# meffmadd/intro-tc-vae

Hardware: AMD Instinct MI355X
Metric: images/sec (64x64x3, z=128, bs=64) intro-TC step (higher is better)
Workload: dtype f32 in/out/accumulate, conv products on split-fp16 MFMA (two scaled fp16 planes, 3 products, fp32-class); 1 GPU; c2: IntroTCSovler.train_step, conv arch, 64x64x3, z_dim=128, channels (64, 128, 256, 512), batch 64/GPU, Adam lr 2e-4, clip 100, N=10000; global_batch=64, parallelism=single, sync_bn=False

## Files before the change

### intro-tc-vae_amd/csrc/conv_igemm.hip

```cpp
#include <float.h>

#include "conv_shared.h"

namespace itcv {



constexpr uint32_t kOobBase = 0x80000000u;

__device__ __forceinline__ float buf_load_s(__amdgpu_buffer_rsrc_t r, uint32_t voff, uint32_t soff) {
  return __builtin_bit_cast(float, __builtin_amdgcn_raw_buffer_load_b32(r, voff, __builtin_amdgcn_readfirstlane(soff), 0));
}

__host__ __device__ inline int tile_rows_for(int M) { return M <= 32 ? 32 : (M <= 64 ? 64 : 128); }

struct ConvArgs {
  const float* x;
  const float* wp;
  const float* bias;
  float* y;
  int B, Ci, H, W, Co;
  int Cip, Mp, N;
  int mt, nt;
  int ktiles, ktiles_per_split, cpt;
// ... 205 lines not shown
    for (int i = 0; i < 8; ++i) {
      const int k = B_KC ? (t & 31) : (t >> 6) + 4 * i, n = B_KC ? (t >> 5) + 8 * i : (t & 63);
      pb[i] = a.B + (long long)min(kb + k, a.K - 1) * a.sbk + (long long)min(n0 + n, a.N - 1) * a.sbn;
    }
#pragma unroll
    for (int i = 0; i < 8; ++i) areg[i] = *pa[i];
#pragma unroll
    for (int i = 0; i < 8; ++i) breg[i] = *pb[i];
    __builtin_amdgcn_sched_group_barrier(0x020, 16, 0);
  };
  auto store_tile = [&](int buf, int kt) {
    const int kb = kt * BK;
#pragma unroll
    for (int i = 0; i < 8; ++i) {
      const int k = A_KC ? (t & 31) : (t >> 6) + 4 * i, m = A_KC ? (t >> 5) + 8 * i : (t & 63);
      As[buf][k * PA + m] = (m0 + m < a.M && kb + k < a.K) ? areg[i] : 0.f;
    }
#pragma unroll
    for (int i = 0; i < 8; ++i) {
      const int k = B_KC ? (t & 31) : (t >> 6) + 4 * i, n = B_KC ? (t >> 5) + 8 * i : (t & 63);
      Bs[buf][k * PB + n] = (n0 + n < a.N && kb + k < a.K) ? breg[i] : 0.f;
    }
  };
  f32x16 acc[1][1];
#pragma unroll
  for (int r = 0; r < 16; ++r) acc[0][0][r] = 0.f;
  if (kt0 < kt1) {
    load_tile(kt0);
    store_tile(0, kt0);
    __syncthreads();
    int cur = 0;
    for (int kt = kt0; kt < kt1; ++kt) {
      const bool more = kt + 1 < kt1;
      if (more) load_tile(kt + 1);
      mfma_tile<BK, PA, PB, 1, 1>(&As[cur][half * PA + wm * 32 + l31], &Bs[cur][half * PB + wn * 32 + l31], acc);
      if (more) store_tile(cur ^ 1, kt + 1);
      __syncthreads();
      cur ^= 1;
    }
  }
  const int n = n0 + wn * 32 + l31;
  if (n >= a.N) return;
  float* out = a.C + (size_t)sk * a.slab_stride;
  const float bv = (a.bias && !a.slab_stride) ? a.bias[n] : 0.f;
#pragma unroll
  for (int r = 0; r < 16; ++r) {
    const int m = m0 + wm * 32 + (r & 3) + 8 * (r >> 2) + 4 * half;
    if (m < a.M) {
      float* q = out + (size_t)m * a.N + n;
      float v = acc[0][0][r] + bv;
      if constexpr (EPI == 1) v = v > 0.f ? v : v * a.slope;
      if constexpr (EPI == 2) v *= a.mask[(long long)m * a.ldm + n] > 0.f ? 1.f : a.slope;
      *q = a.accumulate ? *q + v : v;
    }
  }
}

__global__ void gemm64_reduce(const float* __restrict__ slab, const float* __restrict__ bias, float* __restrict__ C,
                              size_t total, int N, int splits, int accumulate) {
  for (size_t i = (size_t)blockIdx.x * blockDim.x + threadIdx.x; i < total; i += (size_t)gridDim.x * blockDim.x) {
    float s = fold_strided(0.f, slab + i, total, splits);
    if (bias) s += bias[i % N];
    C[i] = accumulate ? C[i] + s : s;
  }
}

template <int EPI>
__global__ void gemm64_reduce_epi(const float* __restrict__ slab, const float* __restrict__ bias, float* __restrict__ C,
                                  size_t total, int N, int splits, const float* __restrict__ mask, long long ldm,
                                  float slope) {
  for (size_t i = (size_t)blockIdx.x * blockDim.x + threadIdx.x; i < total; i += (size_t)gridDim.x * blockDim.x) {
    float s = fold_strided(0.f, slab + i, total, splits);
    if (bias) s += bias[i % N];
    if constexpr (EPI == 1) s = s > 0.f ? s : s * slope;
    if constexpr (EPI == 2) s *= mask[(long long)(i / N) * ldm + (long long)(i % N)] > 0.f ? 1.f : slope;
    C[i] = s;
  }
}

__global__ void pack_weight_kernel(const float* __restrict__ w, float* __restrict__ wp, int Co, int Ci, int KK,
                                   int for_dgrad, int C, int M, int Cip, int Mp) {
  const size_t total = (size_t)KK * Cip * Mp;
  for (size_t i = (size_t)blockIdx.x * blockDim.x + threadIdx.x; i < total; i += (size_t)gridDim.x * blockDim.x) {
    const int k = (int)(i / Mp), m = (int)(i - (size_t)k * Mp);
    const int kt = k >> 4, cib = kt / KK, tap = kt - cib * KK, c = cib * 16 + (k & 15);
    float v = 0.f;
    if (c < C && m < M)
      v = for_dgrad ? w[((size_t)c * Ci + m) * KK + (KK - 1 - tap)] : w[((size_t)m * Ci + c) * KK + tap];
    wp[i] = v;
  }
}


struct ConvArgsB {
  const float* x;
  const u32x4* wp;
  const float* bias;
  float* y;
  int B, Ci, H, W, Co;
  int Mp, N;
  int mt, nt;
  int ktiles, ktiles_per_split, cpt;
  uint32_t x_bytes;
  size_t slab_stride;
#ifdef ITCV_DIAG
  int ablate;
// ... 1376 lines not shown
  if (d.accumulate) {
    if (vec) {
#pragma unroll
      for (int q = 0; q < 9; ++q) {
        const float4 t = reinterpret_cast<const float4*>(dwp)[q];
        tot[4 * q] = t.x, tot[4 * q + 1] = t.y, tot[4 * q + 2] = t.z, tot[4 * q + 3] = t.w;
      }
    } else {
#pragma unroll
      for (int q = 0; q < 36; ++q) tot[q] = dwp[q];
    }
  } else {
#pragma unroll
    for (int q = 0; q < 36; ++q) tot[q] = 0.f;
  }
  for (int k = 0; k < d.nsrc; ++k) {
    const float* p = d.slab[k] + e;
    float acc[36];
#pragma unroll
    for (int q = 0; q < 36; ++q) acc[q] = 0.f;
    int sl = 0;
    for (; sl + 2 <= d.splits[k]; sl += 2) {
      float4 v[2][9];
#pragma unroll
      for (int u = 0; u < 2; ++u)
#pragma unroll
        for (int tp = 0; tp < 9; ++tp) v[u][tp] = *reinterpret_cast<const float4*>(p + (size_t)(sl + u) * stride + (size_t)tp * plane);
#pragma unroll
      for (int u = 0; u < 2; ++u)
#pragma unroll
        for (int tp = 0; tp < 9; ++tp)
          acc[tp] += v[u][tp].x, acc[9 + tp] += v[u][tp].y, acc[18 + tp] += v[u][tp].z, acc[27 + tp] += v[u][tp].w;
    }
    if (sl < d.splits[k]) {
      float4 v[9];
#pragma unroll
      for (int tp = 0; tp < 9; ++tp) v[tp] = *reinterpret_cast<const float4*>(p + (size_t)sl * stride + (size_t)tp * plane);
#pragma unroll
      for (int tp = 0; tp < 9; ++tp) acc[tp] += v[tp].x, acc[9 + tp] += v[tp].y, acc[18 + tp] += v[tp].z, acc[27 + tp] += v[tp].w;
    }
#pragma unroll
    for (int q = 0; q < 36; ++q) tot[q] += acc[q];
  }
  if (vec) {
#pragma unroll
    for (int q = 0; q < 9; ++q) reinterpret_cast<float4*>(dwp)[q] = make_float4(tot[4 * q], tot[4 * q + 1], tot[4 * q + 2], tot[4 * q + 3]);
  } else {
#pragma unroll
    for (int q = 0; q < 36; ++q) dwp[q] = tot[q];
  }
}

constexpr int kWgFineSplits = 64;
__device__ __forceinline__ void wgrad_reduce_tile_fine(const WgReduceDesc& d, int tile, float* part ) {
  const int lane = threadIdx.x & 63, wave = threadIdx.x >> 6, el = lane & 15, sg = wave * 4 + (lane >> 4);
  const int e0 = tile * 16, e = e0 + el;
  const bool live = e < d.coci;
  const size_t plane = (size_t)d.coci, stride = 9 * plane;
  const int o = threadIdx.x;
  const bool oo = o < 144 && e0 * 9 + o < d.coci * 9;
  float tot = (d.accumulate && oo) ? d.dw[(size_t)e0 * 9 + o] : 0.f;
  for (int k = 0; k < d.nsrc; ++k) {
    const int q = (d.splits[k] + 15) >> 4;
    const int s0 = sg * q, s1 = min(s0 + q, d.splits[k]);
    float acc[9];
#pragma unroll
    for (int tp = 0; tp < 9; ++tp) acc[tp] = 0.f;
    if (live) {
      const float* p = d.slab[k] + e;
      int sl = s0;
      for (; sl + 4 <= s1; sl += 4) {
        float v[4][9];
#pragma unroll
        for (int u = 0; u < 4; ++u)
#pragma unroll
          for (int tp = 0; tp < 9; ++tp) v[u][tp] = p[(size_t)(sl + u) * stride + (size_t)tp * plane];
#pragma unroll
        for (int u = 0; u < 4; ++u)
#pragma unroll
          for (int tp = 0; tp < 9; ++tp) acc[tp] += v[u][tp];
      }
      for (; sl < s1; ++sl) {
        float v[9];
#pragma unroll
        for (int tp = 0; tp < 9; ++tp) v[tp] = p[(size_t)sl * stride + (size_t)tp * plane];
#pragma unroll
        for (int tp = 0; tp < 9; ++tp) acc[tp] += v[tp];
      }
    }
    if (k) __syncthreads();
#pragma unroll
    for (int tp = 0; tp < 9; ++tp) part[(sg * 9 + tp) * 16 + el] = acc[tp];
    __syncthreads();
    if (o < 144) {
      const int el2 = o / 9, tp = o - el2 * 9;
      float sum = 0.f;
#pragma unroll
      for (int g = 0; g < 16; ++g) sum += part[(g * 9 + tp) * 16 + el2];
      tot += sum;
    }
  }
  if (oo) d.dw[(size_t)e0 * 9 + o] = tot;
}
static inline bool wgrad_reduce_fine(const int* splits, int nsrc) {
  for (int k = 0; k < nsrc; ++k)
    if (splits[k] >= kWgFineSplits) return true;
  return false;
}
static inline int wgrad_reduce_blocks(int coci, bool fine) { return fine ? cdiv(coci, 16) : cdiv(coci, 1024); }

__global__ __launch_bounds__(256) void wgrad_p_reduce(const float* __restrict__ slab, float* __restrict__ dw, int CoCi,
                                                     int splits, int accumulate, int fine) {
  __shared__ float part[4][9][64];
  WgReduceDesc d;
  d.slab[0] = slab, d.dw = dw, d.splits[0] = splits, d.nsrc = 1, d.coci = CoCi, d.accumulate = accumulate;
  if (fine) wgrad_reduce_tile_fine(d, blockIdx.x, &part[0][0][0]);
  else wgrad_reduce_tile(d, blockIdx.x);
}

constexpr int kWgMaxDesc = 96;
__global__ __launch_bounds__(256) void wgrad_p_reduce_many(const WgReduceDesc* __restrict__ tab, int n, int tile0, int tile1) {
  __shared__ float part[4][9][64];
  __shared__ WgReduceDesc s_desc[kWgMaxDesc];
  {
    const int* src = reinterpret_cast<const int*>(tab);
    int* dst = reinterpret_cast<int*>(s_desc);
    for (int i = threadIdx.x; i < n * (int)(sizeof(WgReduceDesc) / 4); i += blockDim.x) dst[i] = src[i];
  }
  __syncthreads();
  int di = 0;
  for (int t = tile0 + (int)blockIdx.x; t < tile1; t += (int)gridDim.x) {
    while (di + 1 < n && s_desc[di + 1].block0 <= t) ++di;
    const WgReduceDesc d = s_desc[di];
    if (d.fine) {
      wgrad_reduce_tile_fine(d, t - d.block0, &part[0][0][0]);
      __syncthreads();
    } else {
      wgrad_reduce_tile(d, t - d.block0);
    }
  }
}

__global__ __launch_bounds__(256) void splitk_reduce_wgrad_small(const float* __restrict__ slab, float* __restrict__ dw,
                                                                 int Co, int Ci, int KK, int Cip, int cb, int Np,
                                                                 size_t slab_stride, int splits, int accumulate,
                                                                 int swapped) {
  __shared__ float part[16][17];
  const int e = threadIdx.x & 15, g = threadIdx.x >> 4;
  const size_t total = (size_t)Co * Ci * KK, i = (size_t)blockIdx.x * 16 + e;
  float s = 0.f;
  if (i < total) {
    int tap = (int)(i % KK);
    const size_t r = i / KK;
    int ci = (int)(r % Ci), co = (int)(r / Ci);
    if (swapped) {
      const int tmp = ci;
      ci = co, co = tmp, tap = KK - 1 - tap;
    }
    int col;
    if (cb == 128) {
      const int per_tap = Cip / 128;
      col = (tap * per_tap + ci / 128) * 128 + (ci & 127);
    } else {
      const int tpb = 128 / cb;
      col = (tap / tpb) * 128 + (tap % tpb) * cb + ci;
    }
    const float* p = slab + (size_t)co * Np + col;
    for (int k = g; k < splits; k += 16) s += p[(size_t)k * slab_stride];
  }
  part[g][e] = s;
  __syncthreads();
  if (g == 0 && i < total) {
    float t = accumulate ? dw[i] : 0.f;
#pragma unroll
    for (int k = 0; k < 16; ++k) t += part[k][e];
    dw[i] = t;
  }
}

__global__ void splitk_reduce_wgrad(const float* __restrict__ slab, float* __restrict__ dw, int Co, int Ci, int KK,
                                    int Cip, int cb, int Np, size_t slab_stride, int splits, int accumulate,
                                    int swapped) {
  const size_t total = (size_t)Co * Ci * KK;
  for (size_t i = (size_t)blockIdx.x * blockDim.x + threadIdx.x; i < total; i += (size_t)gridDim.x * blockDim.x) {
    int tap = (int)(i % KK);
    const size_t r = i / KK;
    int ci = (int)(r % Ci), co = (int)(r / Ci);
    if (swapped) {
      const int tmp = ci;
      ci = co, co = tmp, tap = KK - 1 - tap;
    }
// ... 684 lines not shown
  ITCV_CHECK_LAUNCH("itcv_conv2d_wgrad_bf16s(reduce)");
  return 0;
}

int itcv_conv2d_wgrad_bf16p_supported(int B, int Ci, int H, int W, int Co, int KS) {
  if (KS != 3 || B <= 0 || Ci < 8 || Co < 8 || (Ci & 7) || (Co & 7)) return 0;
  if (log2_exact(W) < 2 || W > 256 || log2_exact(H) < 0) return 0;
  const long long px = (long long)B * H * W;
  if (px % 64) return 0;
  if (H * W < 64 && 64 % (H * W)) return 0;
  return 1;
}

size_t itcv_conv2d_wgrad_bf16p_workspace(int B, int Ci, int H, int W, int Co, int KS) {
  if (!itcv_conv2d_wgrad_bf16p_supported(B, Ci, H, W, Co, KS)) return 0;
  return plan_wgrad_p(B, Ci, H, W, Co).ws_need;
}

int itcv_conv2d_wgrad_bf16p(const void* xplanes, const void* dyplanes, float* dw, int B, int Ci, int H, int W, int Co,
                            int KS, int up2, int ns, int accumulate, void* ws, size_t ws_bytes, void* stream) {
  if (int e = check_dims("itcv_conv2d_wgrad_bf16p", B, Ci, H, W, Co, KS)) return e;
  ITCV_REQUIRE(xplanes && dyplanes && dw && (ns == 2 || ns == ITCV_PLANES_F16X2), "itcv_conv2d_wgrad_bf16p");
  const int f16 = ns == ITCV_PLANES_F16X2;
  if (!itcv_conv2d_wgrad_bf16p_supported(B, Ci, H, W, Co, KS))
    return fail("%s: shape not supported (KS 3, W a power of two in 4..256, H a power of two, C %% 8)", "itcv_conv2d_wgrad_bf16p");
  if (up2) ITCV_REQUIRE(H % 2 == 0 && W % 2 == 0, "itcv_conv2d_wgrad_bf16p(up2)");
  const WgPlanP p = plan_wgrad_p(B, Ci, H, W, Co);
  if (int e = check_ws("itcv_conv2d_wgrad_bf16p", ws, ws_bytes, p.ws_need)) return e;
  WgradArgsP a;
  a.xp = static_cast<const u32x4*>(xplanes), a.dyp = static_cast<const u32x4*>(dyplanes);
  a.slab = static_cast<float*>(ws);
  a.B = B, a.Ci = Ci, a.H = H, a.W = W, a.Co = Co;
  a.tiles_m = p.tiles_m, a.tiles_n = p.tiles_n;
  a.steps = p.steps, a.steps_per_split = p.sps, a.splits = p.splits;
  a.h_shift = log2_exact(H);
  a.wseg_shift = W > 64 ? log2_exact(W) - 6 : 0;
  a.xplane = (size_t)B * (Ci / 8) * (up2 ? (H / 2) * (W / 2) : H * W);
  a.dyplane = (size_t)B * (Co / 8) * H * W;
  a.xscale = f16 ? reinterpret_cast<const ScaleRec*>(a.xp + 2 * a.xplane) : nullptr;
  a.dyscale = f16 ? reinterpret_cast<const ScaleRec*>(a.dyp + 2 * a.dyplane) : nullptr;
#ifdef ITCV_DIAG
  a.debug = (diag_ablate() & 64) ? 1 : 0;
#endif
  hipStream_t st = S(stream);
  a.groups = p.groups;
  {
    ProfScope prof(st, kProfWgradP, log2_exact(W), p.bm, up2 ? 1 : 0, ns, 2.0 * B * H * W * (double)Co * Ci * KS * KS);
    launch_wgrad_p(a, p, log2_exact(W), up2, f16, st);
  }
  ITCV_CHECK_LAUNCH("itcv_conv2d_wgrad_bf16p");
  if (accumulate == 2) return 0;
  const int coci = Co * Ci;
  const bool fine = wgrad_reduce_fine(&p.slabs, 1);
  hipLaunchKernelGGL(wgrad_p_reduce, dim3(wgrad_reduce_blocks(coci, fine)), dim3(256), 0, st, static_cast<const float*>(ws),
                     dw, coci, p.slabs, accumulate, fine ? 1 : 0);
  ITCV_CHECK_LAUNCH("itcv_conv2d_wgrad_bf16p(reduce)");
  return 0;
}

int itcv_conv2d_wgrad_bf16p_slabs(int B, int Ci, int H, int W, int Co, int KS) {
  if (!itcv_conv2d_wgrad_bf16p_supported(B, Ci, H, W, Co, KS)) return 0;
  return plan_wgrad_p(B, Ci, H, W, Co).slabs;
}
size_t itcv_wgrad_reduce_desc_bytes(void) { return sizeof(WgReduceDesc); }
int itcv_wgrad_reduce_desc(void* host_desc, const float* const* slabs, const int* splits, int nsrc, float* dw, int Co, int Ci,
                           int accumulate, int block0) {
  if (!(host_desc && slabs && splits && nsrc >= 1 && nsrc <= 4 && dw && Co > 0 && Ci > 0 && block0 >= 0)) {
    fail("%s: bad argument (1..4 slab sources, dw, Co/Ci > 0, block0 >= 0)", "itcv_wgrad_reduce_desc");
    return -1;
  }
  WgReduceDesc d;
  memset(&d, 0, sizeof(d));
  for (int k = 0; k < nsrc; ++k) {
    if (!slabs[k] || splits[k] < 1) {
      fail("%s: null slab or non-positive slice count", "itcv_wgrad_reduce_desc");
      return -1;
    }
    d.slab[k] = slabs[k], d.splits[k] = splits[k];
  }
  d.nsrc = nsrc, d.dw = dw, d.coci = Co * Ci, d.accumulate = accumulate ? 1 : 0, d.block0 = block0;
  d.fine = wgrad_reduce_fine(d.splits, nsrc) ? 1 : 0;
  d.nblocks = wgrad_reduce_blocks(d.coci, d.fine != 0);
  memcpy(host_desc, &d, sizeof(d));
  return d.nblocks;
}
int itcv_wgrad_reduce_max_descs(void) { return kWgMaxDesc; }
int itcv_wgrad_reduce_many(const void* dev_table, int n, int total_blocks, void* stream) {
  ITCV_REQUIRE(dev_table && n > 0 && total_blocks > 0, "itcv_wgrad_reduce_many");
  if (n > kWgMaxDesc) return fail("%s: at most %d descriptors per table (itcv_wgrad_reduce_max_descs)", "itcv_wgrad_reduce_many", kWgMaxDesc);
  const int grid = total_blocks < 2048 ? total_blocks : 2048;
  hipLaunchKernelGGL(wgrad_p_reduce_many, dim3(grid), dim3(256), 0, S(stream), static_cast<const WgReduceDesc*>(dev_table), n, 0,
                     total_blocks);
  ITCV_CHECK_LAUNCH("itcv_wgrad_reduce_many");
  return 0;
}

}

namespace itcv {
struct GemmPlan {
  int mt, nt, ktiles, splits, kps;
};
static GemmPlan plan_gemm64(int M, int N, int K) {
  GemmPlan p;
  p.mt = cdiv(M, 64), p.nt = cdiv(N, 64), p.ktiles = cdiv(K, 32);
  const int tiles = p.mt * p.nt;
  int splits = 1;
  if (tiles < 128 && p.ktiles >= 4) {
    splits = cdiv(256, tiles);
    if (splits > 32) splits = 32;
    if (splits > p.ktiles / 2) splits = p.ktiles / 2;
    if (splits < 1) splits = 1;
  }
  p.kps = cdiv(p.ktiles, splits);
  p.splits = cdiv(p.ktiles, p.kps);
  return p;
}
static size_t gemm64_ws(int M, int N, int K) {
  const GemmPlan p = plan_gemm64(M, N, K);
  return p.splits > 1 ? (size_t)p.splits * M * N * sizeof(float) : 0;
}
static int run_gemm64(const char* name, const float* A, const float* B, const float* bias, float* C, int M, int N,
                      int K, long long sam, long long sak, long long sbk, long long sbn, int accumulate, void* ws,
                      size_t ws_bytes, hipStream_t st, int epi = 0, const float* mask = nullptr, long long ldm = 0,
                      float slope = 0.f) {
  const GemmPlan p = plan_gemm64(M, N, K);
  const size_t need = p.splits > 1 ? (size_t)p.splits * M * N * sizeof(float) : 0;
  if (need && (!ws || ws_bytes < need)) return fail("%s: workspace too small (need %lld bytes)", name, (long long)need);
  GemmArgs a;
  a.A = A, a.B = B, a.bias = bias;
  a.C = p.splits > 1 ? static_cast<float*>(ws) : C;
  a.M = M, a.N = N, a.K = K;
  a.sam = sam, a.sak = sak, a.sbk = sbk, a.sbn = sbn;
  a.mt = p.mt, a.nt = p.nt, a.ktiles = p.ktiles, a.ktiles_per_split = p.kps;
  a.slab_stride = p.splits > 1 ? (size_t)M * N : 0;
  a.accumulate = p.splits > 1 ? 0 : accumulate;
  a.mask = mask, a.ldm = ldm, a.slope = slope;
  dim3 grid(p.mt * p.nt, p.splits), blk(256);
  const bool akc = sak == 1, bkc = sbk == 1;
  if (epi == 1 && p.splits == 1) hipLaunchKernelGGL((gemm64_kernel<true, true, 1>), grid, blk, 0, st, a);
  else if (epi == 2 && p.splits == 1) hipLaunchKernelGGL((gemm64_kernel<true, false, 2>), grid, blk, 0, st, a);
  else if (akc && bkc) hipLaunchKernelGGL((gemm64_kernel<true, true>), grid, blk, 0, st, a);
  else if (akc) hipLaunchKernelGGL((gemm64_kernel<true, false>), grid, blk, 0, st, a);
  else if (bkc) hipLaunchKernelGGL((gemm64_kernel<false, true>), grid, blk, 0, st, a);
  else hipLaunchKernelGGL((gemm64_kernel<false, false>), grid, blk, 0, st, a);
  ITCV_CHECK_LAUNCH(name);
  if (p.splits > 1 && epi) {
    const size_t total = (size_t)M * N;
    const dim3 rgrid((int)(cdivz(total, 256) < 1024 ? cdivz(total, 256) : 1024));
    if (epi == 1)
      hipLaunchKernelGGL(gemm64_reduce_epi<1>, rgrid, dim3(256), 0, st, static_cast<const float*>(ws), bias, C, total, N,
                         p.splits, mask, ldm, slope);
    else
      hipLaunchKernelGGL(gemm64_reduce_epi<2>, rgrid, dim3(256), 0, st, static_cast<const float*>(ws), bias, C, total, N,
                         p.splits, mask, ldm, slope);
    ITCV_CHECK_LAUNCH(name);
  } else if (p.splits > 1) {
    const size_t total = (size_t)M * N;
    hipLaunchKernelGGL(gemm64_reduce, dim3((int)(cdivz(total, 256) < 1024 ? cdivz(total, 256) : 1024)), dim3(256), 0, st,
                       static_cast<const float*>(ws), bias, C, total, N, p.splits, accumulate);
    ITCV_CHECK_LAUNCH(name);
  }
  return 0;
}
}

extern "C" {

size_t itcv_linear_workspace(int B, int K, int N) {
  if (B <= 0 || K <= 0 || N <= 0) return 0;
  size_t n = gemm64_ws(B, N, K);
  const size_t d = gemm64_ws(B, K, N), w = gemm64_ws(N, K, B);
  if (d > n) n = d;
  if (w > n) n = w;
  return n;
}
int itcv_linear_fwd(const float* x, const float* w, const float* bias, float* y, int B, int K, int N, void* ws,
                    size_t ws_bytes, void* stream) {
  ITCV_REQUIRE(x && w && y && B > 0 && K > 0 && N > 0, "itcv_linear_fwd");
  return run_gemm64("itcv_linear_fwd", x, w, bias, y, B, N, K, K, 1, 1, K, 0, ws, ws_bytes, S(stream));
}
int itcv_linear_dgrad(const float* dy, const float* w, float* dx, int B, int K, int N, void* ws, size_t ws_bytes,
                      void* stream) {
  ITCV_REQUIRE(dy && w && dx && B > 0 && K > 0 && N > 0, "itcv_linear_dgrad");
  return run_gemm64("itcv_linear_dgrad", dy, w, nullptr, dx, B, K, N, N, 1, K, 1, 0, ws, ws_bytes, S(stream));
}
int itcv_linear_wgrad(const float* dy, const float* x, float* dw, int B, int K, int N, int accumulate, void* ws,
                      size_t ws_bytes, void* stream) {
  ITCV_REQUIRE(dy && x && dw && B > 0 && K > 0 && N > 0, "itcv_linear_wgrad");
  return run_gemm64("itcv_linear_wgrad", dy, x, nullptr, dw, N, K, B, 1, N, K, 1, accumulate, ws, ws_bytes, S(stream));
}

int itcv_linear_lrelu_fwd(const float* x, size_t ldx, const float* w, const float* bias, float* y, int B, int K, int N,
// ... 86 lines not shown
```

### intro-tc-vae_amd/csrc/latent.hip

```cpp
#include <math.h>

#include "common.h"

namespace itcv {

constexpr float kHalfLog2Pi = 0.9189385332046727f;
constexpr float kLog2Pi = 1.8378770664093453f;
constexpr float kVarEps = 1e-4f;
constexpr float kFloor = -50.f;

struct TcConst {
  float lw_n, lw_s, lw_m;
  float log_bn;
  int M;
};

__device__ __forceinline__ float log_iw(const TcConst& c, int jg, int i) {
  if (i == 0) return jg == c.M - 1 ? c.lw_s : c.lw_n;
  return i == 1 ? c.lw_s : c.lw_m;
}

template <bool EPS>
__device__ __forceinline__ float logdens(float d, float lv) {
  if (EPS) {
// ... 159 lines not shown
  __syncthreads();
  float se = 0.f;
  for (int i = tid; i < Bt; i += 256) se += expf(sjoint[(size_t)j * Bt + i] - mx);
  se = block_sum(se, red);
  const float pm = block_sum(prod_acc, red);
  float klj = 0.f;
  if (kk.rows) {
    float a = 0.f;
    for (int l = tid; l < D; l += 256) {
      const float v = kk.lv_loc[(size_t)j * D + l], m = kk.mu_loc[(size_t)j * D + l];
      a += 1.f + v - expf(v) - m * m;
    }
    klj = -0.5f * block_sum(a, red);
  }
  float lcx = 0.f, lpz = 0.f;
  if (ff.rows) {
    float a = 0.f, b = 0.f;
    for (int l = tid; l < D; l += 256) {
      const float zz = ff.z[(size_t)j * D + l];
      a += fmaxf(diag_lp(zz, ff.mu_d[(size_t)j * ff.ld + l], ff.lv_d[(size_t)j * ff.ld + l]), kFloor);
      b += fmaxf(prior_lp(zz), kFloor);
    }
    lcx = block_sum(a, red);
    lpz = block_sum(b, red);
  }
  if (tid == 0) {
    const float lq = mx + logf(se) - (MWS ? c.log_bn : 0.f);
    logqz[j] = lq;
    prodm[j] = pm;
    if (kk.rows) kk.rows[j] = kk.coef_tc * (lq - pm) + kk.coef_kl * klj;
    if (ff.rows) {
      const float mi = lcx - lq, tc = lq - pm, dw = pm - lpz;
      ff.rows[j] = ff.a * mi + ff.b * tc + ff.g * dw;
      if (ff.comps) ff.comps[j] = mi, ff.comps[ff.Bl + j] = tc, ff.comps[2 * ff.Bl + j] = dw;
    }
  }
}

__global__ __launch_bounds__(256) void rows_reduce_kernel(const float* __restrict__ rows, float* __restrict__ out, int B,
                                                         int mean, float scale) {
  __shared__ double red[4];
  double a = 0.0;
  for (int j = threadIdx.x; j < B; j += 256) a += (double)rows[j];
  a = block_sum(a, red);
  if (threadIdx.x == 0) out[0] = scale * (float)(mean ? a / (double)B : a);
}

struct TcGrad {
  const float* g;
  int bcast;
  float coef_tc, coef_kl;
};
__device__ __forceinline__ float tc_g(const TcGrad& t, int j) { return t.bcast ? t.g[0] : t.g[j]; }

__global__ __launch_bounds__(256) void tc_bwd_rows_kernel(
    TcGrad tg, const float* __restrict__ z, const float* __restrict__ mu_all,
    const float* __restrict__ logvar, const float* __restrict__ logqz, const float* __restrict__ lse,
    const float* __restrict__ sjoint, float* __restrict__ wq, float* __restrict__ dz, float* __restrict__ dlogvar, int Bt,
    int row_offset, int D, TcConst c) {
  __shared__ float raz[4][64], rav[4][64];
  const int j = blockIdx.x, jg = row_offset + j, l = blockIdx.y * 64 + (threadIdx.x & 63);
  const int lane = threadIdx.x & 63, wid = threadIdx.x >> 6;
  const bool act = l < D;
  const float gr = tc_g(tg, j), gj = tg.coef_tc * gr, gk = tg.coef_kl * gr, lq = logqz[j];
  const float zj = act ? z[(size_t)j * D + l] : 0.f, lvj = act ? logvar[(size_t)j * D + l] : 0.f;
  const float var = expf(lvj), vh = fmaxf(var, kVarEps), lvh = logf(vh), ivh = 1.f / vh;
  const float ls = act ? lse[(size_t)j * D + l] : 0.f;
  float az = 0.f, av = 0.f;
#pragma unroll 4
  for (int i = wid; i < Bt; i += 4) {
    const float liw = log_iw(c, jg, i);
    const float q = gj * expf(sjoint[(size_t)j * Bt + i] - lq);
    if (blockIdx.y == 0 && lane == 0) wq[(size_t)j * Bt + i] = q;
    if (act) {
      const float d = zj - mu_all[(size_t)i * D + l];
      const float lp = -(0.5f * (lvh + d * d * ivh) + kHalfLog2Pi);
      if (lp >= kFloor) {
        const float G = q - gj * expf(lp + liw - ls);
        const float dv = d * ivh;
        az -= G * dv;
        av -= G * 0.5f * (ivh - dv * dv);
      }
    }
  }
  raz[wid][lane] = az, rav[wid][lane] = av;
  __syncthreads();
  if (wid == 0 && act) {
    dz[(size_t)j * D + l] = (raz[0][lane] + raz[1][lane]) + (raz[2][lane] + raz[3][lane]);
    const float dl = ((rav[0][lane] + rav[1][lane]) + (rav[2][lane] + rav[3][lane])) * var;
    dlogvar[(size_t)j * D + l] = gk != 0.f ? dl + gk * (-0.5f) * (1.f - var) : dl;
  }
}

__global__ __launch_bounds__(256) void tc_bwd_cols_kernel(
    TcGrad tg, const float* __restrict__ z, const float* __restrict__ mu_all,
    const float* __restrict__ logvar, const float* __restrict__ lse, const float* __restrict__ wq,
    float* __restrict__ dmu_all, int Bl, int Bt, int row_offset, int D, TcConst c) {
  __shared__ float racc[4][64];
  const int i = blockIdx.x, l = blockIdx.y * 64 + (threadIdx.x & 63);
  const int lane = threadIdx.x & 63, wid = threadIdx.x >> 6;
  const bool act = l < D;
  const float mi = act ? mu_all[(size_t)i * D + l] : 0.f;
  float acc = 0.f;
#pragma unroll 2
  for (int j = wid; j < Bl; j += 4) {
    const float gj = tg.coef_tc * tc_g(tg, j), q = wq[(size_t)j * Bt + i], liw = log_iw(c, row_offset + j, i);
    if (act) {
      const float vh = fmaxf(expf(logvar[(size_t)j * D + l]), kVarEps), ivh = 1.f / vh;
      const float d = z[(size_t)j * D + l] - mi;
      const float lp = -(0.5f * (logf(vh) + d * d * ivh) + kHalfLog2Pi);
      if (lp >= kFloor) acc += (q - gj * expf(lp + liw - lse[(size_t)j * D + l])) * d * ivh;
    }
  }
  racc[wid][lane] = acc;
  __syncthreads();
  if (wid == 0 && act) {
    float v = (racc[0][lane] + racc[1][lane]) + (racc[2][lane] + racc[3][lane]);
    if (tg.coef_kl != 0.f && i >= row_offset && i < row_offset + Bl) v += tg.coef_kl * tc_g(tg, i - row_offset) * mi;
    dmu_all[(size_t)i * D + l] = v;
  }
}

struct TcFullGrad {
  const float* g;
  int bcast;
  float a, cq, cp, c;
};
__device__ __forceinline__ float tcf_g(const TcFullGrad& t, int j) { return t.bcast ? t.g[0] : t.g[j]; }

__global__ __launch_bounds__(256) void tc_full_bwd_rows_kernel(
    TcFullGrad tg, const float* __restrict__ z, const float* __restrict__ mu_all, const float* __restrict__ lv_all, int ld,
    const float* __restrict__ ivar, const float* __restrict__ logqz, const float* __restrict__ lse,
    const float* __restrict__ sjoint, float* __restrict__ wq, float* __restrict__ dz, int Bt, int row_offset, int D,
    TcConst c) {
  __shared__ float raz[4][64];
  const int j = blockIdx.x, jg = row_offset + j, l = blockIdx.y * 64 + (threadIdx.x & 63);
  const int lane = threadIdx.x & 63, wid = threadIdx.x >> 6;
  const bool act = l < D;
  const float gr = tcf_g(tg, j), cq = tg.cq * gr, cp = tg.cp * gr, lq = logqz[j];
  const float zj = act ? z[(size_t)j * D + l] : 0.f, ls = act ? lse[(size_t)j * D + l] : 0.f;
  float az = 0.f;
#pragma unroll 4
  for (int i = wid; i < Bt; i += 4) {
    const float liw = log_iw(c, jg, i);
    const float q = cq * expf(sjoint[(size_t)j * Bt + i] - lq);
    if (blockIdx.y == 0 && lane == 0) wq[(size_t)j * Bt + i] = q;
    if (act) {
      const float d = zj - mu_all[(size_t)i * ld + l], iv = ivar[(size_t)i * D + l];
      const float lp = -0.5f * (lv_all[(size_t)i * ld + l] + d * d * iv) - kHalfLog2Pi;
      if (lp >= kFloor) az -= (q + cp * expf(lp + liw - ls)) * d * iv;
    }
  }
  raz[wid][lane] = az;
  __syncthreads();
  if (wid == 0 && act) {
    float v = (raz[0][lane] + raz[1][lane]) + (raz[2][lane] + raz[3][lane]);
    const float m = mu_all[(size_t)jg * ld + l], lv = lv_all[(size_t)jg * ld + l], d = zj - m;
    if (diag_lp(zj, m, lv) >= kFloor) v += tg.a * gr * (-d * expf(-lv));
    if (prior_lp(zj) >= kFloor) v += tg.c * gr * zj;
    dz[(size_t)j * D + l] = v;
  }
}

__global__ __launch_bounds__(256) void tc_full_bwd_cols_kernel(
// ... 577 lines not shown
```

Before: 4309 images/s.

## Vectorize gemm64 and wgrad fine reduce, cost-sort reduce work, batch TC-backward loads

Adds a float4-loading gemm64 variant with a 4-deep register prefetch ring and an LDS-staged, vectorized epilogue, used when pointers and strides are 16-byte aligned. The fine wgrad reduction now handles 64 elements per block with float4 loads. The multi-descriptor reduce kernel orders its work items by estimated cost, largest first. The TC backward row and column kernels hoist 16 iterations of global loads into registers before computing, to expose memory-level parallelism. Together these aim to cut load instruction count and latency stalls, at the cost of more registers and LDS and some extra work on clamped out-of-range lanes.

```diff
diff --git a/intro-tc-vae_amd/csrc/conv_igemm.hip b/intro-tc-vae_amd/csrc/conv_igemm.hip
--- a/intro-tc-vae_amd/csrc/conv_igemm.hip
+++ b/intro-tc-vae_amd/csrc/conv_igemm.hip
@@ -281,6 +281,127 @@
       if constexpr (EPI == 1) v = v > 0.f ? v : v * a.slope;
       if constexpr (EPI == 2) v *= a.mask[(long long)m * a.ldm + n] > 0.f ? 1.f : a.slope;
       *q = a.accumulate ? *q + v : v;
+    }
+  }
+}
+
+template <bool A_KC, bool B_KC, int EPI = 0>
+__global__ __launch_bounds__(256) void gemm64_vec_kernel(GemmArgs a) {
+  constexpr int BM = 64, BN = 64, BK = 32, PA = BM + 1, PB = BN + 1, NS = 4;
+  static_assert(2 * BK * PA >= BM * PB, "the C tile is staged in As");
+  __shared__ float As[2][BK * PA];
+  __shared__ float Bs[2][BK * PB];
+  const int t = threadIdx.x, lane = t & 63, wid = t >> 6;
+  const int wm = wid >> 1, wn = wid & 1, l31 = lane & 31, half = lane >> 5;
+  const int tile_m = blockIdx.x % a.mt, tile_n = blockIdx.x / a.mt, sk = blockIdx.y;
+  const int m0 = tile_m * BM, n0 = tile_n * BN;
+  const int kt0 = sk * a.ktiles_per_split, kt1 = min(a.ktiles, kt0 + a.ktiles_per_split);
+  const int ak = A_KC ? (t & 7) * 4 : (t >> 4), am = A_KC ? (t >> 3) : (t & 15) * 4;
+  const int bk = B_KC ? (t & 7) * 4 : (t >> 4), bn = B_KC ? (t >> 3) : (t & 15) * 4;
+  constexpr int AKI = A_KC ? 0 : 16, AMI = A_KC ? 32 : 0, BKI = B_KC ? 0 : 16, BNI = B_KC ? 32 : 0;
+
+  float4 ra[NS][2], rb[NS][2];
+  auto load_tile = [&](int kt, float4 (&pa)[2], float4 (&pb)[2]) {
+    const int kb = kt * BK;
+#pragma unroll
+    for (int i = 0; i < 2; ++i) {
+      const int k = kb + ak + i * AKI, m = m0 + am + i * AMI;
+      const float* p = A_KC ? a.A + (long long)min(m, a.M - 1) * a.sam + min(k, a.K - 4)
+                            : a.A + (long long)min(k, a.K - 1) * a.sak + min(m, a.M - 4);
+      pa[i] = *reinterpret_cast<const float4*>(p);
+    }
+#pragma unroll
+    for (int i = 0; i < 2; ++i) {
+      const int k = kb + bk + i * BKI, n = n0 + bn + i * BNI;
+      const float* p = B_KC ? a.B + (long long)min(n, a.N - 1) * a.sbn + min(k, a.K - 4)
+                            : a.B + (long long)min(k, a.K - 1) * a.sbk + min(n, a.N - 4);
+      pb[i] = *reinterpret_cast<const float4*>(p);
+    }
+    __builtin_amdgcn_sched_group_barrier(0x020, 4, 0);
+  };
+  auto store_tile = [&](int buf, int kt, const float4 (&pa)[2], const float4 (&pb)[2]) {
+    const int kb = kt * BK;
+#pragma unroll
+    for (int i = 0; i < 2; ++i) {
+      const int k = ak + i * AKI, m = am + i * AMI;
+      const bool ok = m0 + m < a.M && kb + k < a.K;
+      const float v[4] = {ok ? pa[i].x : 0.f, ok ? pa[i].y : 0.f, ok ? pa[i].z : 0.f, ok ? pa[i].w : 0.f};
+#pragma unroll
+      for (int j = 0; j < 4; ++j) As[buf][A_KC ? (k + j) * PA + m : k * PA + m + j] = v[j];
+    }
+#pragma unroll
+    for (int i = 0; i < 2; ++i) {
+      const int k = bk + i * BKI, n = bn + i * BNI;
+      const bool ok = n0 + n < a.N && kb + k < a.K;
+      const float v[4] = {ok ? pb[i].x : 0.f, ok ? pb[i].y : 0.f, ok ? pb[i].z : 0.f, ok ? pb[i].w : 0.f};
+#pragma unroll
+      for (int j = 0; j < 4; ++j) Bs[buf][B_KC ? (k + j) * PB + n : k * PB + n + j] = v[j];
+    }
+  };
+  f32x16 acc[1][1];
+#pragma unroll
+  for (int r = 0; r < 16; ++r) acc[0][0][r] = 0.f;
+  if (kt0 < kt1) {
+#pragma unroll
+    for (int s = 0; s < NS; ++s) load_tile(min(kt0 + s, kt1 - 1), ra[s], rb[s]);
+    store_tile(0, kt0, ra[0], rb[0]);
+    __syncthreads();
+    int cur = 0, kt = kt0;
+    auto step = [&](auto sc) {
+      constexpr int s = decltype(sc)::value;
+      load_tile(min(kt + NS, kt1 - 1), ra[s], rb[s]);
+      mfma_tile<BK, PA, PB, 1, 1>(&As[cur][half * PA + wm * 32 + l31], &Bs[cur][half * PB + wn * 32 + l31], acc);
+      if (kt + 1 < kt1) store_tile(cur ^ 1, kt + 1, ra[(s + 1) % NS], rb[(s + 1) % NS]);
+      __syncthreads();
+      cur ^= 1;
+      return ++kt < kt1;
+    };
+    while (step(std::integral_constant<int, 0>{}) && step(std::integral_constant<int, 1>{}) &&
+           step(std::integral_constant<int, 2>{}) && step(std::integral_constant<int, 3>{})) {
+    }
+    static_assert(NS == 4, "the ring is walked by four written-out steps");
+  }
+  float* Cs = &As[0][0];
+#pragma unroll
+  for (int r = 0; r < 16; ++r)
+    Cs[(wm * 32 + (r & 3) + 8 * (r >> 2) + 4 * half) * PB + wn * 32 + l31] = acc[0][0][r];
+  __syncthreads();
+  float* out = a.C + (size_t)sk * a.slab_stride;
+  const int n = n0 + (t & 15) * 4, nc = min(n, a.N - 4);
+  float bv[4] = {0.f, 0.f, 0.f, 0.f};
+  if (a.bias && !a.slab_stride) {
+#pragma unroll
+    for (int j = 0; j < 4; ++j) bv[j] = a.bias[nc + j];
+  }
+  float4 old[4];
+#pragma unroll
+  for (int i = 0; i < 4; ++i) old[i] = make_float4(0.f, 0.f, 0.f, 0.f);
+  if (a.accumulate) {
+#pragma unroll
+    for (int i = 0; i < 4; ++i)
+      old[i] = *reinterpret_cast<const float4*>(out + (size_t)min(m0 + (t >> 4) + 16 * i, a.M - 1) * a.N + nc);
+  }
+  float mk[4][4];
+  if constexpr (EPI == 2) {
+#pragma unroll
+    for (int i = 0; i < 4; ++i)
+#pragma unroll
+      for (int j = 0; j < 4; ++j) mk[i][j] = a.mask[(long long)min(m0 + (t >> 4) + 16 * i, a.M - 1) * a.ldm + nc + j];
+  }
+#pragma unroll
+  for (int i = 0; i < 4; ++i) {
+    const int row = (t >> 4) + 16 * i, m = m0 + row;
+    if (m < a.M && n < a.N) {
+      const float o4[4] = {old[i].x, old[i].y, old[i].z, old[i].w};
+      float v[4];
+#pragma unroll
+      for (int j = 0; j < 4; ++j) {
+        v[j] = Cs[row * PB + (t & 15) * 4 + j] + bv[j];
+        if constexpr (EPI == 1) v[j] = v[j] > 0.f ? v[j] : v[j] * a.slope;
+        if constexpr (EPI == 2) v[j] *= mk[i][j] > 0.f ? 1.f : a.slope;
+        if (a.accumulate) v[j] = o4[j] + v[j];
+      }
+      *reinterpret_cast<float4*>(out + (size_t)m * a.N + n) = make_float4(v[0], v[1], v[2], v[3]);
     }
   }
 }
@@ -1763,55 +1884,72 @@
 }
 
 constexpr int kWgFineSplits = 64;
-__device__ __forceinline__ void wgrad_reduce_tile_fine(const WgReduceDesc& d, int tile, float* part ) {
-  const int lane = threadIdx.x & 63, wave = threadIdx.x >> 6, el = lane & 15, sg = wave * 4 + (lane >> 4);
-  const int e0 = tile * 16, e = e0 + el;
+constexpr int kWgFineTiles = 4;
+constexpr int kWgFineElems = 16 * kWgFineTiles, kWgFineOut = 9 * kWgFineElems;
+constexpr int kWgPartFloats = 16 * kWgFineOut;
+static_assert(kWgFineElems == 64 && kWgFineOut <= 3 * 256, "lane mapping of wgrad_reduce_tile_fine");
+
+template <int U>
+__device__ __forceinline__ void wgrad_fine_add(float (&acc)[36], const float* p, int sl, size_t stride, size_t plane) {
+  float4 v[U][9];
+#pragma unroll
+  for (int u = 0; u < U; ++u)
+#pragma unroll
+    for (int tp = 0; tp < 9; ++tp) v[u][tp] = *reinterpret_cast<const float4*>(p + (size_t)(sl + u) * stride + (size_t)tp * plane);
+#pragma unroll
+  for (int u = 0; u < U; ++u)
+#pragma unroll
+    for (int tp = 0; tp < 9; ++tp)
+      acc[tp] += v[u][tp].x, acc[9 + tp] += v[u][tp].y, acc[18 + tp] += v[u][tp].z, acc[27 + tp] += v[u][tp].w;
+}
+
+__device__ __forceinline__ void wgrad_reduce_tile_fine(const WgReduceDesc& d, int item, float* part ) {
+  const int lane = threadIdx.x & 63, wave = threadIdx.x >> 6, el4 = lane & 15, sg = wave * 4 + (lane >> 4);
+  const int e0 = item * kWgFineElems, e = e0 + el4 * 4;
   const bool live = e < d.coci;
   const size_t plane = (size_t)d.coci, stride = 9 * plane;
-  const int o = threadIdx.x;
-  const bool oo = o < 144 && e0 * 9 + o < d.coci * 9;
-  float tot = (d.accumulate && oo) ? d.dw[(size_t)e0 * 9 + o] : 0.f;
+  const int nout = min(kWgFineOut, (d.coci - e0) * 9);
+  float* dwp = d.dw + (size_t)e0 * 9;
+  float tot[3];
+#pragma unroll
+  for (int r = 0; r < 3; ++r) {
+    const int o = (int)threadIdx.x + 256 * r;
+    tot[r] = (d.accumulate && o < nout) ? dwp[o] : 0.f;
+  }
   for (int k = 0; k < d.nsrc; ++k) {
     const int q = (d.splits[k] + 15) >> 4;
     const int s0 = sg * q, s1 = min(s0 + q, d.splits[k]);
-    float acc[9];
-#pragma unroll
-    for (int tp = 0; tp < 9; ++tp) acc[tp] = 0.f;
+    float acc[36];
+#pragma unroll
+    for (int f = 0; f < 36; ++f) acc[f] = 0.f;
     if (live) {
       const float* p = d.slab[k] + e;
       int sl = s0;
-      for (; sl + 4 <= s1; sl += 4) {
-        float v[4][9];
-#pragma unroll
-        for (int u = 0; u < 4; ++u)
-#pragma unroll
-          for (int tp = 0; tp < 9; ++tp) v[u][tp] = p[(size_t)(sl + u) * stride + (size_t)tp * plane];
-#pragma unroll
-        for (int u = 0; u < 4; ++u)
-#pragma unroll
-          for (int tp = 0; tp < 9; ++tp) acc[tp] += v[u][tp];
+      for (; sl + 4 <= s1; sl += 4) wgrad_fine_add<4>(acc, p, sl, stride, plane);
+      if (sl + 2 <= s1) wgrad_fine_add<2>(acc, p, sl, stride, plane), sl += 2;
+      if (sl < s1) wgrad_fine_add<1>(acc, p, sl, stride, plane);
+    }
+    if (k) __syncthreads();
+    float4* pw = reinterpret_cast<float4*>(part + sg * kWgFineOut + el4 * 36);
+#pragma unroll
+    for (int c = 0; c < 9; ++c) pw[c] = make_float4(acc[4 * c], acc[4 * c + 1], acc[4 * c + 2], acc[4 * c + 3]);
+    __syncthreads();
+#pragma unroll
+    for (int r = 0; r < 3; ++r) {
+      const int o = (int)threadIdx.x + 256 * r;
+      if (o < kWgFineOut) {
+        float sum = 0.f;
+#pragma unroll
+        for (int g = 0; g < 16; ++g) sum += part[g * kWgFineOut + o];
+        tot[r] += sum;
       }
-      for (; sl < s1; ++sl) {
-        float v[9];
-#pragma unroll
-        for (int tp = 0; tp < 9; ++tp) v[tp] = p[(size_t)sl * stride + (size_t)tp * plane];
-#pragma unroll
-        for (int tp = 0; tp < 9; ++tp) acc[tp] += v[tp];
-      }
-    }
-    if (k) __syncthreads();
-#pragma unroll
-    for (int tp = 0; tp < 9; ++tp) part[(sg * 9 + tp) * 16 + el] = acc[tp];
-    __syncthreads();
-    if (o < 144) {
-      const int el2 = o / 9, tp = o - el2 * 9;
-      float sum = 0.f;
-#pragma unroll
-      for (int g = 0; g < 16; ++g) sum += part[(g * 9 + tp) * 16 + el2];
-      tot += sum;
-    }
-  }
-  if (oo) d.dw[(size_t)e0 * 9 + o] = tot;
+    }
+  }
+#pragma unroll
+  for (int r = 0; r < 3; ++r) {
+    const int o = (int)threadIdx.x + 256 * r;
+    if (o < nout) dwp[o] = tot[r];
+  }
 }
 static inline bool wgrad_reduce_fine(const int* splits, int nsrc) {
   for (int k = 0; k < nsrc; ++k)
@@ -1822,32 +1960,57 @@
 
 __global__ __launch_bounds__(256) void wgrad_p_reduce(const float* __restrict__ slab, float* __restrict__ dw, int CoCi,
                                                      int splits, int accumulate, int fine) {
-  __shared__ float part[4][9][64];
+  __shared__ __attribute__((aligned(16))) float part[kWgPartFloats];
   WgReduceDesc d;
   d.slab[0] = slab, d.dw = dw, d.splits[0] = splits, d.nsrc = 1, d.coci = CoCi, d.accumulate = accumulate;
-  if (fine) wgrad_reduce_tile_fine(d, blockIdx.x, &part[0][0][0]);
+  if (fine) wgrad_reduce_tile_fine(d, blockIdx.x, part);
   else wgrad_reduce_tile(d, blockIdx.x);
 }
 
 constexpr int kWgMaxDesc = 96;
-__global__ __launch_bounds__(256) void wgrad_p_reduce_many(const WgReduceDesc* __restrict__ tab, int n, int tile0, int tile1) {
-  __shared__ float part[4][9][64];
+__device__ __forceinline__ int wgrad_desc_items(const WgReduceDesc& d) {
+  return d.fine ? (d.nblocks + kWgFineTiles - 1) / kWgFineTiles : d.nblocks;
+}
+__global__ __launch_bounds__(256) void wgrad_p_reduce_many(const WgReduceDesc* __restrict__ tab, int n) {
+  __shared__ __attribute__((aligned(16))) float part[kWgPartFloats];
   __shared__ WgReduceDesc s_desc[kWgMaxDesc];
+  __shared__ int s_cost[kWgMaxDesc], s_items[kWgMaxDesc], s_ord[kWgMaxDesc], s_first[kWgMaxDesc + 1];
+  const int tid = threadIdx.x;
   {
     const int* src = reinterpret_cast<const int*>(tab);
     int* dst = reinterpret_cast<int*>(s_desc);
-    for (int i = threadIdx.x; i < n * (int)(sizeof(WgReduceDesc) / 4); i += blockDim.x) dst[i] = src[i];
+    for (int i = tid; i < n * (int)(sizeof(WgReduceDesc) / 4); i += blockDim.x) dst[i] = src[i];
   }
   __syncthreads();
-  int di = 0;
-  for (int t = tile0 + (int)blockIdx.x; t < tile1; t += (int)gridDim.x) {
-    while (di + 1 < n && s_desc[di + 1].block0 <= t) ++di;
-    const WgReduceDesc d = s_desc[di];
+  if (tid < n) {
+    const WgReduceDesc& d = s_desc[tid];
+    int slices = 0;
+    for (int k = 0; k < d.nsrc; ++k) slices += d.splits[k];
+    s_cost[tid] = slices * (d.fine ? kWgFineElems : 1024);
+    s_items[tid] = wgrad_desc_items(d);
+  }
+  __syncthreads();
+  if (tid < n) {
+    const int mine = s_cost[tid];
+    int rank = 0, first = 0;
+    for (int j = 0; j < n; ++j) {
+      const int cj = s_cost[j];
+      if (cj > mine || (cj == mine && j < tid)) ++rank, first += s_items[j];
+    }
+    s_ord[rank] = tid, s_first[rank] = first;
+    if (rank == n - 1) s_first[n] = first + s_items[tid];
+  }
+  __syncthreads();
+  const int total = s_first[n];
+  int r = 0;
+  for (int w = (int)blockIdx.x; w < total; w += (int)gridDim.x) {
+    while (s_first[r + 1] <= w) ++r;
+    const WgReduceDesc& d = s_desc[s_ord[r]];
     if (d.fine) {
-      wgrad_reduce_tile_fine(d, t - d.block0, &part[0][0][0]);
+      wgrad_reduce_tile_fine(d, w - s_first[r], part);
       __syncthreads();
     } else {
-      wgrad_reduce_tile(d, t - d.block0);
+      wgrad_reduce_tile(d, w - s_first[r]);
     }
   }
 }
@@ -2638,7 +2801,8 @@
   if (accumulate == 2) return 0;
   const int coci = Co * Ci;
   const bool fine = wgrad_reduce_fine(&p.slabs, 1);
-  hipLaunchKernelGGL(wgrad_p_reduce, dim3(wgrad_reduce_blocks(coci, fine)), dim3(256), 0, st, static_cast<const float*>(ws),
+  const int rblocks = fine ? cdiv(wgrad_reduce_blocks(coci, true), kWgFineTiles) : wgrad_reduce_blocks(coci, false);
+  hipLaunchKernelGGL(wgrad_p_reduce, dim3(rblocks), dim3(256), 0, st, static_cast<const float*>(ws),
                      dw, coci, p.slabs, accumulate, fine ? 1 : 0);
   ITCV_CHECK_LAUNCH("itcv_conv2d_wgrad_bf16p(reduce)");
   return 0;
@@ -2675,8 +2839,7 @@
   ITCV_REQUIRE(dev_table && n > 0 && total_blocks > 0, "itcv_wgrad_reduce_many");
   if (n > kWgMaxDesc) return fail("%s: at most %d descriptors per table (itcv_wgrad_reduce_max_descs)", "itcv_wgrad_reduce_many", kWgMaxDesc);
   const int grid = total_blocks < 2048 ? total_blocks : 2048;
-  hipLaunchKernelGGL(wgrad_p_reduce_many, dim3(grid), dim3(256), 0, S(stream), static_cast<const WgReduceDesc*>(dev_table), n, 0,
-                     total_blocks);
+  hipLaunchKernelGGL(wgrad_p_reduce_many, dim3(grid), dim3(256), 0, S(stream), static_cast<const WgReduceDesc*>(dev_table), n);
   ITCV_CHECK_LAUNCH("itcv_wgrad_reduce_many");
   return 0;
 }
@@ -2724,7 +2887,17 @@
   a.mask = mask, a.ldm = ldm, a.slope = slope;
   dim3 grid(p.mt * p.nt, p.splits), blk(256);
   const bool akc = sak == 1, bkc = sbk == 1;
-  if (epi == 1 && p.splits == 1) hipLaunchKernelGGL((gemm64_kernel<true, true, 1>), grid, blk, 0, st, a);
+  const auto al16 = [](const void* q) { return (reinterpret_cast<uintptr_t>(q) & 15) == 0; };
+  const bool vec = al16(A) && al16(B) && al16(a.C) && N % 4 == 0 &&
+                   (akc ? (K % 4 == 0 && sam % 4 == 0) : (sam == 1 && M % 4 == 0 && sak % 4 == 0)) &&
+                   (bkc ? (K % 4 == 0 && sbn % 4 == 0) : (sbn == 1 && sbk % 4 == 0));
+  if (vec && epi == 1 && p.splits == 1) hipLaunchKernelGGL((gemm64_vec_kernel<true, true, 1>), grid, blk, 0, st, a);
+  else if (vec && epi == 2 && p.splits == 1) hipLaunchKernelGGL((gemm64_vec_kernel<true, false, 2>), grid, blk, 0, st, a);
+  else if (vec && akc && bkc) hipLaunchKernelGGL((gemm64_vec_kernel<true, true>), grid, blk, 0, st, a);
+  else if (vec && akc) hipLaunchKernelGGL((gemm64_vec_kernel<true, false>), grid, blk, 0, st, a);
+  else if (vec && bkc) hipLaunchKernelGGL((gemm64_vec_kernel<false, true>), grid, blk, 0, st, a);
+  else if (vec) hipLaunchKernelGGL((gemm64_vec_kernel<false, false>), grid, blk, 0, st, a);
+  else if (epi == 1 && p.splits == 1) hipLaunchKernelGGL((gemm64_kernel<true, true, 1>), grid, blk, 0, st, a);
   else if (epi == 2 && p.splits == 1) hipLaunchKernelGGL((gemm64_kernel<true, false, 2>), grid, blk, 0, st, a);
   else if (akc && bkc) hipLaunchKernelGGL((gemm64_kernel<true, true>), grid, blk, 0, st, a);
   else if (akc) hipLaunchKernelGGL((gemm64_kernel<true, false>), grid, blk, 0, st, a);
diff --git a/intro-tc-vae_amd/csrc/latent.hip b/intro-tc-vae_amd/csrc/latent.hip
--- a/intro-tc-vae_amd/csrc/latent.hip
+++ b/intro-tc-vae_amd/csrc/latent.hip
@@ -235,6 +235,7 @@
   float coef_tc, coef_kl;
 };
 __device__ __forceinline__ float tc_g(const TcGrad& t, int j) { return t.bcast ? t.g[0] : t.g[j]; }
+constexpr int kTcBwdU = 16;
 
 __global__ __launch_bounds__(256) void tc_bwd_rows_kernel(
     TcGrad tg, const float* __restrict__ z, const float* __restrict__ mu_all,
@@ -250,19 +251,30 @@
   const float var = expf(lvj), vh = fmaxf(var, kVarEps), lvh = logf(vh), ivh = 1.f / vh;
   const float ls = act ? lse[(size_t)j * D + l] : 0.f;
   float az = 0.f, av = 0.f;
-#pragma unroll 4
-  for (int i = wid; i < Bt; i += 4) {
-    const float liw = log_iw(c, jg, i);
-    const float q = gj * expf(sjoint[(size_t)j * Bt + i] - lq);
-    if (blockIdx.y == 0 && lane == 0) wq[(size_t)j * Bt + i] = q;
-    if (act) {
-      const float d = zj - mu_all[(size_t)i * D + l];
-      const float lp = -(0.5f * (lvh + d * d * ivh) + kHalfLog2Pi);
-      if (lp >= kFloor) {
-        const float G = q - gj * expf(lp + liw - ls);
-        const float dv = d * ivh;
-        az -= G * dv;
-        av -= G * 0.5f * (ivh - dv * dv);
+  const int lc = min(l, D - 1);
+  for (int i0 = wid; i0 < Bt; i0 += 4 * kTcBwdU) {
+    float mv[kTcBwdU], sv[kTcBwdU];
+#pragma unroll
+    for (int u = 0; u < kTcBwdU; ++u) {
+      const int ic = min(i0 + 4 * u, Bt - 1);
+      mv[u] = mu_all[(size_t)ic * D + lc];
+      sv[u] = sjoint[(size_t)j * Bt + ic];
+    }
+#pragma unroll
+    for (int u = 0; u < kTcBwdU; ++u) {
+      const int i = i0 + 4 * u;
+      if (i < Bt) {
+        const float liw = log_iw(c, jg, i);
+        const float q = gj * expf(sv[u] - lq);
+        if (blockIdx.y == 0 && lane == 0) wq[(size_t)j * Bt + i] = q;
+        const float d = zj - mv[u];
+        const float lp = -(0.5f * (lvh + d * d * ivh) + kHalfLog2Pi);
+        if (act && lp >= kFloor) {
+          const float G = q - gj * expf(lp + liw - ls);
+          const float dv = d * ivh;
+          az -= G * dv;
+          av -= G * 0.5f * (ivh - dv * dv);
+        }
       }
     }
   }
@@ -285,14 +297,28 @@
   const bool act = l < D;
   const float mi = act ? mu_all[(size_t)i * D + l] : 0.f;
   float acc = 0.f;
-#pragma unroll 2
-  for (int j = wid; j < Bl; j += 4) {
-    const float gj = tg.coef_tc * tc_g(tg, j), q = wq[(size_t)j * Bt + i], liw = log_iw(c, row_offset + j, i);
-    if (act) {
-      const float vh = fmaxf(expf(logvar[(size_t)j * D + l]), kVarEps), ivh = 1.f / vh;
-      const float d = z[(size_t)j * D + l] - mi;
-      const float lp = -(0.5f * (logf(vh) + d * d * ivh) + kHalfLog2Pi);
-      if (lp >= kFloor) acc += (q - gj * expf(lp + liw - lse[(size_t)j * D + l])) * d * ivh;
+  const int lc = min(l, D - 1);
+  for (int j0 = wid; j0 < Bl; j0 += 4 * kTcBwdU) {
+    float lvv[kTcBwdU], zv[kTcBwdU], lsv[kTcBwdU], qv[kTcBwdU], gv[kTcBwdU];
+#pragma unroll
+    for (int u = 0; u < kTcBwdU; ++u) {
+      const int jc = min(j0 + 4 * u, Bl - 1);
+      lvv[u] = logvar[(size_t)jc * D + lc];
+      zv[u] = z[(size_t)jc * D + lc];
+      lsv[u] = lse[(size_t)jc * D + lc];
+      qv[u] = wq[(size_t)jc * Bt + i];
+      gv[u] = tg.g[tg.bcast ? 0 : jc];
+    }
+#pragma unroll
+    for (int u = 0; u < kTcBwdU; ++u) {
+      const int j = j0 + 4 * u;
+      if (j < Bl) {
+        const float gj = tg.coef_tc * gv[u], q = qv[u], liw = log_iw(c, row_offset + j, i);
+        const float vh = fmaxf(expf(lvv[u]), kVarEps), ivh = 1.f / vh;
+        const float d = zv[u] - mi;
+        const float lp = -(0.5f * (logf(vh) + d * d * ivh) + kHalfLog2Pi);
+        if (act && lp >= kFloor) acc += (q - gj * expf(lp + liw - lsv[u])) * d * ivh;
+      }
     }
   }
   racc[wid][lane] = acc;
```

Result: faster. 4356 images/s (median of 6 runs) (+1.1%).
